# marl/l3embedding

Hardware: AMD Instinct MI355X
Metric: AVC training pairs/sec (1s audio + 224x224 frame) (higher is better)
Workload: dtype f32; 1 GPU; full cnn_L3_melspec2 AVC training step (audio+vision+fusion, fwd+bwd+Adam), batch 64 per GPU, global batch 64, fp32, inputs resident in HBM; global_batch=64, parallelism=dp1, fp32_conv=f4x4

## Files before the change

l3embedding_amd/csrc/conv_wgrad_bx6.hip:

```cpp
#include "kernels.h"
#include "device_common.h"
#include "wgw_common.h"

#include <stdlib.h>

#include <mutex>
#include <type_traits>

namespace l3 {

namespace {

template <int V>
using IC = std::integral_constant<int, V>;

__device__ __forceinline__ unsigned hi16_pair(unsigned a, unsigned b) { return __builtin_amdgcn_perm(b, a, 0x07060302u); }

struct Split3 {
    unsigned h, m, l;
};
__device__ __forceinline__ Split3 split_pair(float a, float b) {
    const unsigned ua = __builtin_bit_cast(unsigned, a), ub = __builtin_bit_cast(unsigned, b);
    Split3 s;
    s.h = hi16_pair(ua, ub);
    const float ra = a - __builtin_bit_cast(float, ua & 0xffff0000u), rb = b - __builtin_bit_cast(float, ub & 0xffff0000u);
    const unsigned va = __builtin_bit_cast(unsigned, ra), vb = __builtin_bit_cast(unsigned, rb);
    s.m = hi16_pair(va, vb);
    const float qa = ra - __builtin_bit_cast(float, va & 0xffff0000u), qb = rb - __builtin_bit_cast(float, vb & 0xffff0000u);
    s.l = hi16_pair(__builtin_bit_cast(unsigned, qa), __builtin_bit_cast(unsigned, qb));
    return s;
}

__device__ __forceinline__ f32x2 lds_pair(unsigned addr) {
    return *reinterpret_cast<const __attribute__((address_space(3))) f32x2*>((uintptr_t)addr);
}

template <int UC>
struct WgbGeom : WgwGeom<UC> {
    using G = WgwGeom<UC>;
    static constexpr int UNIT_BYTES = G::STAGE;
    static constexpr int STAGE2 = 2 * UNIT_BYTES;
    static constexpr unsigned BUF1 = 0x10000;
    static constexpr size_t LDS_BYTES = BUF1 + (size_t)STAGE2;
    static_assert(STAGE2 <= 0x10000, "stage buffer");
    static constexpr int PIECES2 = 2 * G::PIECES;
    static constexpr int PER_WAVE = (PIECES2 + 7) / 8;
    __host__ __device__ static constexpr int tr(int j) { return UC == 8 ? 0 : UC == 4 ? j >> 2 : j >> 1; }
    __host__ __device__ static constexpr int tc(int j) { return UC == 8 ? j : UC == 4 ? j & 3 : j & 1; }
};

template <int UC>
__global__ __launch_bounds__(512) void conv_wgrad_bx6_kernel(WgwArgs a) {
    using G = WgbGeom<UC>;
    constexpr int UR = G::UR, XPITCH = G::XPITCH, YPITCH = G::YPITCH, PER_WAVE = G::PER_WAVE;
    extern __shared__ __attribute__((aligned(16))) char smem[];

    const int t = threadIdx.x;
    const int wave = __builtin_amdgcn_readfirstlane(t >> 6), lane_id = t & 63;
    const int tiles = a.ctiles * a.ktiles;
    const int logical = xcd_remap(blockIdx.x, tiles * a.splits);
    const int sp = logical / tiles, tile = logical - sp * tiles;
    const int ct = tile / a.ktiles, kt = tile - ct * a.ktiles;
    const int c0 = ct * 64, k0 = kt * 64;
    const int u_begin = sp * a.per_split, u_end = min(a.units, u_begin + a.per_split);
    const int nunits = max(0, u_end - u_begin), nstage = (nunits + 1) >> 1;

    const int y_last = 2 * UR * (a.uy - 1), x_last = 2 * UC * (a.ux - 1);
    const size_t xshift = (size_t)(a.W + 1) * a.Cin * 4;
    const __amdgpu_buffer_rsrc_t xsrd = __builtin_amdgcn_make_buffer_rsrc(
        (void*)(reinterpret_cast<const char*>(a.x) - xshift), 0, (int)((size_t)a.N * a.H * a.W * a.Cin * 4 + xshift), 0x00020000);
    const __amdgpu_buffer_rsrc_t ysrd =
        __builtin_amdgcn_make_buffer_rsrc((void*)a.dy, 0, (int)((size_t)a.N * a.H * a.W * a.Cout * 4), 0x00020000);
    const int per_img = a.uy * a.ux;

    int q_u = u_begin;
    int q_n = u_begin / per_img, q_y = (u_begin - q_n * per_img) / a.ux, q_x = u_begin - q_n * per_img - q_y * a.ux;
    auto issue = [&](int s) __attribute__((always_inline)) {
        char* S = smem + (s & 1) * G::BUF1;
        int xbv[2], ybv[2];
        unsigned flg[2], dead[2];
#pragma unroll
        for (int h = 0; h < 2; ++h) {
            const int Y0 = 2 * UR * q_y, X0 = 2 * UC * q_x;
            xbv[h] = ((q_n * a.H + Y0) * a.W + X0) * a.Cin * 4;
            ybv[h] = ((q_n * a.H + Y0) * a.W + X0) * a.Cout * 4;
            flg[h] = (unsigned)(1 - min(q_y, 1)) | (unsigned)(1 - min(a.uy - 1 - q_y, 1)) << 1 | (unsigned)(1 - min(q_x, 1)) << 2 |
                     (unsigned)(1 - min(a.ux - 1 - q_x, 1)) << 3;
            dead[h] = q_u < u_end ? 0u : 0x80000000u;
            ++q_u;
            if (++q_x == a.ux) {
                q_x = 0;
                if (++q_y == a.uy) {
                    q_y = 0;
                    ++q_n;
                }
            }
        }
        int lane = lane_id;
        asm volatile("" : "+v"(lane));
#pragma unroll
        for (int q = 0; q < PER_WAVE; ++q) {
            const int pi = wave + 8 * q;
            if (pi < G::PIECES2) {
                const int h = pi >= G::PIECES ? 1 : 0;
                const int piece = pi - h * G::PIECES;
                const bool isx = piece < G::XPIECES;
                const int pix = (isx ? piece : piece - G::XPIECES) * 4 + (lane >> 4);
                const int py = isx ? pix / XPITCH : pix / YPITCH, px = isx ? pix - py * XPITCH : pix - py * YPITCH;
                const int ry = py - (isx ? 1 : 0), rx = px - (isx ? 1 : 0);
                const unsigned f = h ? flg[1] : flg[0];
                const unsigned out = ((f & 1u) & (unsigned)(ry < 0)) | ((f >> 1 & 1u) & (unsigned)(y_last + ry >= a.H)) |
                                     ((f >> 2 & 1u) & (unsigned)(rx < 0)) | ((f >> 3 & 1u) & (unsigned)(x_last + rx >= a.W)) |
                                     (unsigned)(isx && pix >= G::XPIX);
                const unsigned vo = (unsigned)((py * a.W + px) * (isx ? a.Cin : a.Cout) * 4 + (isx ? c0 : k0) * 4 + (lane & 15) * 16) |
                                    (out << 31) | (h ? dead[1] : dead[0]);
                auto* dst = (__attribute__((address_space(3))) void*)(S + h * G::UNIT_BYTES + piece * 1024);
                if (isx)
                    __builtin_amdgcn_raw_ptr_buffer_load_lds(xsrd, dst, 16, (int)vo, h ? xbv[1] : xbv[0], 0, 0);
                else
                    __builtin_amdgcn_raw_ptr_buffer_load_lds(ysrd, dst, 16, (int)vo, h ? ybv[1] : ybv[0], 0, 0);
            }
        }
    };

    const int l31 = lane_id & 31, grp = lane_id >> 5;
    const unsigned lds0 = (unsigned)(uintptr_t)smem;
    const unsigned lane_base = lds0 + (unsigned)(grp * G::UNIT_BYTES + l31 * 8);

    const int xi = wave >> 1;
    const int nuA = (wave & 1) ? 3 : 0, nuB = (wave & 1) ? 2 : 1;
    auto sgpr = [](float v) { return __builtin_bit_cast(float, __builtin_amdgcn_readfirstlane(__builtin_bit_cast(int, v))); };
    auto bt_a = [](int x) { return x == 0 ? 0 : x == 2 ? 2 : 1; };
    auto bt_b = [](int x) { return x == 0 ? 2 : x == 1 ? 2 : x == 2 ? 1 : 3; };
    const int ra = bt_a(xi), rb = bt_b(xi);
    const float sa = sgpr(xi == 1 ? 1.f : -1.f);
    const float sbA = sgpr(nuA == 1 ? 1.f : -1.f), sbB = sgpr(nuB == 1 ? 1.f : -1.f);
    const float r1 = sgpr(xi == 1 ? 1.f : -1.f), c1B = sgpr(nuB == 1 ? 1.f : -1.f);
    const int ry0 = xi == 3 ? 1 : 0, cy0A = nuA == 3 ? 1 : 0;
    auto xadr = [&](int r, int c) { return lane_base + (unsigned)((r * XPITCH + c) * 256); };
    auto yadr = [&](int r, int c) { return lane_base + (unsigned)(G::XBYTES + (r * YPITCH + c) * 256); };
    unsigned xA[4] = {xadr(ra, bt_a(nuA)), xadr(rb, bt_a(nuA)), xadr(ra, bt_b(nuA)), xadr(rb, bt_b(nuA))};
    unsigned xB[4] = {xadr(ra, bt_a(nuB)), xadr(rb, bt_a(nuB)), xadr(ra, bt_b(nuB)), xadr(rb, bt_b(nuB))};
    unsigned yA[2] = {yadr(ry0, cy0A), yadr(1, cy0A)};
    unsigned yB[4] = {yadr(ry0, 0), yadr(ry0, 1), yadr(1, 0), yadr(1, 1)};
    asm volatile("" : "+v"(xA[0]), "+v"(xA[1]), "+v"(xA[2]), "+v"(xA[3]), "+v"(xB[0]), "+v"(xB[1]), "+v"(xB[2]), "+v"(xB[3]));
    asm volatile("" : "+v"(yA[0]), "+v"(yA[1]), "+v"(yB[0]), "+v"(yB[1]), "+v"(yB[2]), "+v"(yB[3]));

    f32x16 acc[2][2][2];
#pragma unroll
    for (int pp = 0; pp < 2; ++pp)
#pragma unroll
        for (int i = 0; i < 2; ++i)
#pragma unroll
            for (int jn = 0; jn < 2; ++jn)
#pragma unroll
                for (int r = 0; r < 16; ++r) acc[pp][i][jn][r] = 0.f;

    auto run = [&](auto NRT, auto GRP) __attribute__((always_inline)) {
        constexpr int NR = decltype(NRT)::value;
        u32x4 Ah[2], Am[2], Al[2], Bh, Bm, Bl;
        auto lds_f = [](unsigned addr) { return *reinterpret_cast<const __attribute__((address_space(3))) float*>((uintptr_t)addr); };

        auto build_b = [&](auto PP, auto JN, unsigned buf) __attribute__((always_inline)) {
            constexpr int pp = decltype(PP)::value, jn = decltype(JN)::value;
            float z[2];
#pragma unroll
            for (int j = 0; j < 8; ++j) {
                if (!(j & 3)) __builtin_amdgcn_sched_barrier(0);
                const int tt = j & 1, tp = j >> 1;
                const unsigned yo = (unsigned)(((2 * G::tr(j)) * YPITCH + 2 * G::tc(j)) * 256 + 4 * jn);
                float zz;
                if constexpr (pp == 0) {
                    zz = lds_f(yA[0] + yo);
                    if constexpr (NR == 2) zz = fmaf(r1, lds_f(yA[1] + yo), zz);
                } else {
                    zz = fmaf(c1B, lds_f(yB[1] + yo), lds_f(yB[0] + yo));
                    if constexpr (NR == 2) zz = fmaf(r1, fmaf(c1B, lds_f(yB[3] + yo), lds_f(yB[2] + yo)), zz);
                }
                z[tt] = zz;
                if (tt == 1) {
                    const Split3 sz = split_pair(z[0], z[1]);
                    Bh[tp] = sz.h; Bm[tp] = sz.m; Bl[tp] = sz.l;
                }
            }
            __builtin_amdgcn_sched_barrier(0);
        };
        auto operands = [&](auto PP, unsigned buf) __attribute__((always_inline)) {
            constexpr int pp = decltype(PP)::value;
            const float sb = pp ? sbB : sbA;
            float v[2][2];
#pragma unroll
            for (int j = 0; j < 8; ++j) {
                if (!(j & 1)) __builtin_amdgcn_sched_barrier(0);
                const int tt = j & 1, tp = j >> 1;
                const unsigned xo = (unsigned)(((2 * G::tr(j)) * XPITCH + 2 * G::tc(j)) * 256);
                const f32x2 xa = lds_pair((pp ? xB[0] : xA[0]) + xo), xb = lds_pair((pp ? xB[1] : xA[1]) + xo);
                const f32x2 xc = lds_pair((pp ? xB[2] : xA[2]) + xo), xd = lds_pair((pp ? xB[3] : xA[3]) + xo);
#pragma unroll
                for (int e = 0; e < 2; ++e) v[tt][e] = fmaf(sb, fmaf(sa, xd[e], xc[e]), fmaf(sa, xb[e], xa[e]));
                if (tt == 1) {
#pragma unroll
                    for (int e = 0; e < 2; ++e) {
                        const Split3 sv = split_pair(v[0][e], v[1][e]);
                        Ah[e][tp] = sv.h; Am[e][tp] = sv.m; Al[e][tp] = sv.l;
                    }
                }
            }
            build_b(PP, IC<0>{}, buf);
        };
        auto multiply = [&](auto PP, unsigned buf) __attribute__((always_inline)) {
            constexpr int pp = decltype(PP)::value;
#pragma unroll
            for (int jn = 0; jn < 2; ++jn) {
                if (jn == 1) build_b(PP, IC<1>{}, buf);
                const bf16x8 bh = __builtin_bit_cast(bf16x8, Bh), bm = __builtin_bit_cast(bf16x8, Bm), bl = __builtin_bit_cast(bf16x8, Bl);
                const bf16x8 ah0 = __builtin_bit_cast(bf16x8, Ah[0]), am0 = __builtin_bit_cast(bf16x8, Am[0]), al0 = __builtin_bit_cast(bf16x8, Al[0]);
                const bf16x8 ah1 = __builtin_bit_cast(bf16x8, Ah[1]), am1 = __builtin_bit_cast(bf16x8, Am[1]), al1 = __builtin_bit_cast(bf16x8, Al[1]);
                f32x16 d0 = acc[pp][0][jn], d1 = acc[pp][1][jn];
                d0 = __builtin_amdgcn_mfma_f32_32x32x16_bf16(al0, bh, d0, 0, 0, 0);
                d1 = __builtin_amdgcn_mfma_f32_32x32x16_bf16(al1, bh, d1, 0, 0, 0);
                d0 = __builtin_amdgcn_mfma_f32_32x32x16_bf16(ah0, bl, d0, 0, 0, 0);
                d1 = __builtin_amdgcn_mfma_f32_32x32x16_bf16(ah1, bl, d1, 0, 0, 0);
                d0 = __builtin_amdgcn_mfma_f32_32x32x16_bf16(am0, bm, d0, 0, 0, 0);
                d1 = __builtin_amdgcn_mfma_f32_32x32x16_bf16(am1, bm, d1, 0, 0, 0);
                d0 = __builtin_amdgcn_mfma_f32_32x32x16_bf16(am0, bh, d0, 0, 0, 0);
                d1 = __builtin_amdgcn_mfma_f32_32x32x16_bf16(am1, bh, d1, 0, 0, 0);
                d0 = __builtin_amdgcn_mfma_f32_32x32x16_bf16(ah0, bm, d0, 0, 0, 0);
                d1 = __builtin_amdgcn_mfma_f32_32x32x16_bf16(ah1, bm, d1, 0, 0, 0);
                d0 = __builtin_amdgcn_mfma_f32_32x32x16_bf16(ah0, bh, d0, 0, 0, 0);
                d1 = __builtin_amdgcn_mfma_f32_32x32x16_bf16(ah1, bh, d1, 0, 0, 0);
                acc[pp][0][jn] = d0;
                acc[pp][1][jn] = d1;
                __builtin_amdgcn_sched_barrier(0);
            }
        };
        auto barrier = [] {
            __builtin_amdgcn_sched_barrier(0);
            __builtin_amdgcn_s_barrier();
            __builtin_amdgcn_sched_barrier(0);
        };
        auto wait_all = [] { asm volatile("s_waitcnt vmcnt(0)" ::: "memory"); };
        constexpr bool grp_o = decltype(GRP)::value != 0;
        if constexpr (grp_o) barrier();
        for (int c = 0; c < nstage; ++c) {
            const unsigned buf = 0;
            operands(IC<0>{}, buf);
            barrier();
            issue(c + 1);
            multiply(IC<0>{}, buf);
            barrier();
            operands(IC<1>{}, buf);
            if constexpr (grp_o) wait_all();
            barrier();
            multiply(IC<1>{}, buf);
            if constexpr (!grp_o) wait_all();
            barrier();
#pragma unroll
            for (int k = 0; k < 4; ++k) {
                xA[k] ^= G::BUF1;
                xB[k] ^= G::BUF1;
                yB[k] ^= G::BUF1;
            }
            yA[0] ^= G::BUF1;
            yA[1] ^= G::BUF1;
        }
        if constexpr (!grp_o) barrier();
    };
    {
        issue(0);
        asm volatile("s_waitcnt vmcnt(0)" ::: "memory");
        __syncthreads();
        const bool two_rows = xi == 1 || xi == 2;
        if (wave < 4) {
            if (two_rows) run(IC<2>{}, IC<0>{}); else run(IC<1>{}, IC<0>{});
        } else {
            if (two_rows) run(IC<2>{}, IC<1>{}); else run(IC<1>{}, IC<1>{});
        }
        asm volatile("s_waitcnt vmcnt(0)" ::: "memory");
    }

    int l31s = l31, grps = grp;
    asm volatile("" : "+v"(l31s), "+v"(grps));
#pragma unroll
    for (int pp = 0; pp < 2; ++pp) {
        const int nu = pp ? nuB : nuA;
        const float w00 = (xi == 3 ? -1.f : 1.f) * (nu == 3 ? -1.f : 1.f);
        float* out = a.part + ((size_t)(sp * 16 + xi * 4 + nu) * a.Cin + c0 + 8 * grps) * a.Cout + k0 + 2 * l31s;
#pragma unroll
        for (int i = 0; i < 2; ++i)
#pragma unroll
            for (int r = 0; r < 16; ++r) {
                const int c = 2 * ((r & 3) + 8 * (r >> 2)) + i;
                __builtin_nontemporal_store(f32x2{w00 * acc[pp][i][0][r], w00 * acc[pp][i][1][r]},
                                            reinterpret_cast<f32x2*>(out + (size_t)c * a.Cout));
            }
    }
}

template <int UC>
void launch_wgb(const WgwArgs& a, hipStream_t s) {
    using G = WgbGeom<UC>;
    static std::once_flag once[L3_MAX_DEVICES];
    int dev = 0;
    (void)hipGetDevice(&dev);
    std::call_once(once[dev & (L3_MAX_DEVICES - 1)], [] {
        (void)hipFuncSetAttribute((const void*)conv_wgrad_bx6_kernel<UC>, hipFuncAttributeMaxDynamicSharedMemorySize, (int)G::LDS_BYTES);
    });
    hipLaunchKernelGGL((conv_wgrad_bx6_kernel<UC>), dim3(a.ctiles * a.ktiles * a.splits), dim3(512), G::LDS_BYTES, s, a);
}

}

void conv_wgrad_bx6_launch(const WgwArgs& a, int uc, hipStream_t s) {
    if (uc == 8)
        launch_wgb<8>(a, s);
    else if (uc == 4)
        launch_wgb<4>(a, s);
    else
        launch_wgb<2>(a, s);
}

}
```

l3embedding_amd/csrc/conv_wgrad_wino.hip:

```cpp
#include "kernels.h"
#include "device_common.h"
#include "wgw_common.h"

#include <stdlib.h>

#include <mutex>

namespace l3 {

namespace {

__device__ __forceinline__ f32x2 lds_f32x2(unsigned lds_offset) {
    const f32x2 v = *reinterpret_cast<const __attribute__((address_space(3))) f32x2*>((uintptr_t)lds_offset);
    asm volatile("");
    return v;
}

__device__ __forceinline__ f32x2 pk_fma(f32x2 c, f32x2 x, f32x2 y) {
    asm("v_pk_fma_f32 %0, %1, %2, %0" : "+v"(y) : "s"(c), "v"(x));
    return y;
}
__device__ __forceinline__ f32x2 pk_fma_w(f32x2 c, f32x2 x, f32x2 y) {
    asm("v_pk_fma_f32 %0, %1, %2, %0\n\ts_nop 3" : "+v"(y) : "s"(c), "v"(x));
    return y;
}
template <int UC>
__global__ __launch_bounds__(1024) void conv_wgrad_wino_kernel(WgwArgs a) {
    using G = WgwGeom<UC>;
    constexpr int UR = G::UR, XPITCH = G::XPITCH, YPITCH = G::YPITCH;
    extern __shared__ __attribute__((aligned(16))) char smem[];

    const int t = threadIdx.x;
    const int wave = __builtin_amdgcn_readfirstlane(t >> 6), lane = t & 63;
    const int tiles = a.ctiles * a.ktiles;
    const int logical = xcd_remap(blockIdx.x, tiles * a.splits);
    const int sp = logical / tiles, tile = logical - sp * tiles;
    const int ct = tile / a.ktiles, kt = tile - ct * a.ktiles;
    const int c0 = ct * 64, k0 = kt * 64;
    const int u_begin = sp * a.per_split, u_end = min(a.units, u_begin + a.per_split);

    unsigned pc_voff[2], pc_out[2];
    bool pc_isx[2];
    const int y_last = 2 * UR * (a.uy - 1), x_last = 2 * UC * (a.ux - 1);
#pragma unroll
    for (int q = 0; q < 2; ++q) {
        const int piece = wave + 16 * q;
        const bool isx = piece < G::XPIECES;
        const int pix = (isx ? piece : piece - G::XPIECES) * 4 + (lane >> 4);
        const int pitch = isx ? XPITCH : YPITCH;
        const int py = pix / pitch, px = pix - py * pitch;
        const int C = isx ? a.Cin : a.Cout;
        const int ry = py - (isx ? 1 : 0), rx = px - (isx ? 1 : 0);
        pc_isx[q] = isx;
        pc_voff[q] = (unsigned)((py * a.W + px) * C * 4 + (isx ? c0 : k0) * 4 + (lane & 15) * 16);
        unsigned out = 0;
#pragma unroll
        for (int cls = 0; cls < 16; ++cls) {
            const int rc = cls >> 2, cc = cls & 3;
            const bool bad = ((rc & 1) && ry < 0) || ((rc & 2) && y_last + ry >= a.H) || ((cc & 1) && rx < 0) ||
                             ((cc & 2) && x_last + rx >= a.W) || (isx && pix >= G::XPIX);
            out |= bad ? 1u << cls : 0u;
        }
        pc_out[q] = out;
    }
    const bool second = wave + 16 < G::PIECES;
    const size_t xshift = (size_t)(a.W + 1) * a.Cin * 4;
    const __amdgpu_buffer_rsrc_t xsrd = __builtin_amdgcn_make_buffer_rsrc(
        (void*)(reinterpret_cast<const char*>(a.x) - xshift), 0, (int)((size_t)a.N * a.H * a.W * a.Cin * 4 + xshift), 0x00020000);
    const __amdgpu_buffer_rsrc_t ysrd =
        __builtin_amdgcn_make_buffer_rsrc((void*)a.dy, 0, (int)((size_t)a.N * a.H * a.W * a.Cout * 4), 0x00020000);

    const int per_img = a.uy * a.ux;
    int un = u_begin / per_img;
    int uyi = (u_begin - un * per_img) / a.ux;
    int uxi = u_begin - un * per_img - uyi * a.ux;

    auto issue = [&](int buf) {
        const int Y0 = 2 * UR * uyi, X0 = 2 * UC * uxi;
        const int xbase = ((un * a.H + Y0) * a.W + X0) * a.Cin * 4;
        const int ybase = ((un * a.H + Y0) * a.W + X0) * a.Cout * 4;
        const int rcls = (1 - min(uyi, 1)) + 2 * (1 - min(a.uy - 1 - uyi, 1)), ccls = (1 - min(uxi, 1)) + 2 * (1 - min(a.ux - 1 - uxi, 1));
        const int cls = rcls * 4 + ccls;
        char* S = smem + buf * G::STAGE;
#pragma unroll
        for (int q = 0; q < 2; ++q) {
            if (q == 1 && !second) break;
            const unsigned vo = (__builtin_amdgcn_ubfe(pc_out[q], (unsigned)cls, 1u) << 31) | pc_voff[q];
            if (pc_isx[q])
                __builtin_amdgcn_raw_ptr_buffer_load_lds(xsrd, (__attribute__((address_space(3))) void*)(S + (wave + 16 * q) * 1024),
                                                         16, (int)vo, xbase, 0, 0);
            else
                __builtin_amdgcn_raw_ptr_buffer_load_lds(ysrd, (__attribute__((address_space(3))) void*)(S + (wave + 16 * q) * 1024),
                                                         16, (int)vo, ybase, 0, 0);
        }
        if (++uxi == a.ux) {
            uxi = 0;
            if (++uyi == a.uy) {
                uyi = 0;
                ++un;
            }
        }
    };

    const int xi = wave >> 2, nu = (wave + (wave >> 2)) & 3;
    const int ra = xi == 0 ? 0 : xi == 2 ? 2 : 1, rb = xi == 0 ? 2 : xi == 1 ? 2 : xi == 2 ? 1 : 3;
    const int ca = nu == 0 ? 0 : nu == 2 ? 2 : 1, cb = nu == 0 ? 2 : nu == 1 ? 2 : nu == 2 ? 1 : 3;
    auto sgpr = [](float v) { return __builtin_bit_cast(float, __builtin_amdgcn_readfirstlane(__builtin_bit_cast(int, v))); };
    const float sa = sgpr(xi == 1 ? 1.f : -1.f), sb = sgpr(nu == 1 ? 1.f : -1.f);
    const int nr = (xi == 0 || xi == 3) ? 1 : 2, nc = (nu == 0 || nu == 3) ? 1 : 2;
    const int ry0 = xi == 3 ? 1 : 0, cy0 = nu == 3 ? 1 : 0;
    const float sr0 = xi == 3 ? -1.f : 1.f, sr1 = xi == 2 ? -1.f : 1.f;
    const float sc0 = nu == 3 ? -1.f : 1.f, sc1 = nu == 2 ? -1.f : 1.f;
    const float w00 = sgpr(sr0 * sc0), w01 = sgpr(sr0 * sc1), w10 = sgpr(sr1 * sc0), w11 = sgpr(sr1 * sc1);
    const f32x2 sa2 = {sa, sa}, sb2 = {sb, sb}, w01_2 = {w01 * w00, w01 * w00}, w10_2 = {w10 * w00, w10 * w00},
                w11_2 = {w11 * w00, w11 * w00};

    const int l31 = lane & 31, half = lane >> 5;
    const int ltr = G::lane_tr(half), ltc = G::lane_tc(half);
    auto xaddr = [&](int r, int c) { return ((r + 2 * ltr) * XPITCH + c + 2 * ltc) * 256 + l31 * 8; };
    auto yaddr = [&](int r, int c) { return G::XBYTES + ((r + 2 * ltr) * YPITCH + c + 2 * ltc) * 256 + l31 * 8; };
    const int x_aa = xaddr(ra, ca), x_ba = xaddr(rb, ca), x_ab = xaddr(ra, cb), x_bb = xaddr(rb, cb);
    const int y_00 = yaddr(ry0, cy0), y_01 = yaddr(ry0, 1), y_10 = yaddr(1, cy0), y_11 = yaddr(1, 1);
    const unsigned lds0 = (unsigned)(uintptr_t)smem;
    unsigned p_aa = lds0 + x_aa, p_ba = lds0 + x_ba, p_ab = lds0 + x_ab, p_bb = lds0 + x_bb;
    unsigned q_00 = lds0 + y_00, q_01 = lds0 + y_01, q_10 = lds0 + y_10, q_11 = lds0 + y_11;
    asm volatile("" : "+v"(p_aa), "+v"(p_ba), "+v"(p_ab), "+v"(p_bb), "+v"(q_00), "+v"(q_01), "+v"(q_10), "+v"(q_11));

    f32x16 acc[2][2];
#pragma unroll
    for (int i = 0; i < 2; ++i)
#pragma unroll
        for (int jn = 0; jn < 2; ++jn)
#pragma unroll
            for (int r = 0; r < 16; ++r) acc[i][jn][r] = 0.f;

    struct Raw {
        f32x2 x[4], y[4];
    };
    auto run = [&](auto NRT, auto NCT) {
    constexpr int NR = decltype(NRT)::value, NC = decltype(NCT)::value;
    auto load_raw = [&](int sb, auto JT, Raw& r, const Raw& prev) {
        constexpr int j = decltype(JT)::value;
        constexpr bool share = NC == 1 && j > 0 && G::imm_tr(j) == G::imm_tr(j > 0 ? j - 1 : 0) &&
                               G::imm_tc(j) == G::imm_tc(j > 0 ? j - 1 : 0) + 1;
        const int ix = ((2 * G::imm_tr(j)) * XPITCH + 2 * G::imm_tc(j)) * 256;
        const int iy = ((2 * G::imm_tr(j)) * YPITCH + 2 * G::imm_tc(j)) * 256;
        f32x2 xa, xb;
        if constexpr (share) {
            xa = prev.x[2];
            xb = prev.x[3];
        } else {
            xa = lds_f32x2(p_aa + sb + ix);
            xb = lds_f32x2(p_ba + sb + ix);
        }
        const f32x2 xc = lds_f32x2(p_ab + sb + ix), xd = lds_f32x2(p_bb + sb + ix);
        f32x2 ya = lds_f32x2(q_00 + sb + iy), yb = ya, yc = ya, yd = ya;
        if (NC == 2) yb = lds_f32x2(q_01 + sb + iy);
        if (NR == 2) yc = lds_f32x2(q_10 + sb + iy);
        if (NR == 2 && NC == 2) yd = lds_f32x2(q_11 + sb + iy);
        r.x[0] = xa; r.x[1] = xb; r.x[2] = xc; r.x[3] = xd;
        r.y[0] = ya; r.y[1] = yb; r.y[2] = yc; r.y[3] = yd;
    };
    auto mfma_step = [&](const Raw& r) {
        const f32x2 v = pk_fma_w(sb2, pk_fma(sa2, r.x[3], r.x[2]), pk_fma(sa2, r.x[1], r.x[0]));
        f32x2 z;
        if constexpr (NR == 1 && NC == 1) {
            z = r.y[0];
        } else if constexpr (NR == 1) {
            z = pk_fma_w(w01_2, r.y[1], r.y[0]);
        } else if constexpr (NC == 1) {
            z = pk_fma_w(w10_2, r.y[2], r.y[0]);
        } else {
            z = pk_fma_w(w11_2, r.y[3], pk_fma(w10_2, r.y[2], pk_fma(w01_2, r.y[1], r.y[0])));
        }
#pragma unroll
        for (int i = 0; i < 2; ++i)
#pragma unroll
            for (int jn = 0; jn < 2; ++jn) acc[i][jn] = __builtin_amdgcn_mfma_f32_32x32x2f32(v[i], z[jn], acc[i][jn], 0, 0, 0);
    };
    auto compute = [&](auto BUF) {
        constexpr int S = decltype(BUF)::value * G::STAGE;
        Raw r0, r1;
        load_raw(S, std::integral_constant<int, 0>{}, r0, r0);
        __builtin_amdgcn_sched_barrier(0);
        load_raw(S, std::integral_constant<int, 1>{}, r1, r0);
        mfma_step(r0);
        __builtin_amdgcn_sched_barrier(0);
        load_raw(S, std::integral_constant<int, 2>{}, r0, r1);
        mfma_step(r1);
        __builtin_amdgcn_sched_barrier(0);
        load_raw(S, std::integral_constant<int, 3>{}, r1, r0);
        mfma_step(r0);
        __builtin_amdgcn_sched_barrier(0);
        mfma_step(r1);
    };
    auto stage_barrier = [&]() {
        __builtin_amdgcn_sched_barrier(0);
        __syncthreads();
        __builtin_amdgcn_sched_barrier(0);
    };

    const int nunits = u_end - u_begin;
    if (nunits > 0) {
        issue(0);
        __syncthreads();
        for (int u = 0; u < nunits; u += 2) {
            if (u + 1 < nunits) issue(1);
            compute(std::integral_constant<int, 0>{});
            stage_barrier();
            if (u + 1 < nunits) {
                if (u + 2 < nunits) issue(0);
                compute(std::integral_constant<int, 1>{});
                stage_barrier();
            }
        }
    }
    };
    if (nr == 1 && nc == 1)
        run(std::integral_constant<int, 1>{}, std::integral_constant<int, 1>{});
    else if (nr == 1)
        run(std::integral_constant<int, 1>{}, std::integral_constant<int, 2>{});
    else if (nc == 1)
        run(std::integral_constant<int, 2>{}, std::integral_constant<int, 1>{});
    else
        run(std::integral_constant<int, 2>{}, std::integral_constant<int, 2>{});

    float* out = a.part + ((size_t)(sp * 16 + xi * 4 + nu) * a.Cin + c0) * a.Cout + k0;
#pragma unroll
    for (int i = 0; i < 2; ++i)
#pragma unroll
        for (int r = 0; r < 16; ++r) {
            const int c = 2 * ((r & 3) + 8 * (r >> 2) + 4 * half) + i;
            __builtin_nontemporal_store(f32x2{w00 * acc[i][0][r], w00 * acc[i][1][r]}, reinterpret_cast<f32x2*>(out + (size_t)c * a.Cout + 2 * l31));
        }
}

__global__ __launch_bounds__(256) void wgw_finish_kernel(const float* __restrict__ part, float* __restrict__ dw, int cc,
                                                         int splits) {
    const int idx = blockIdx.x * 256 + threadIdx.x;
    if (idx >= cc) return;
    float u[16];
#pragma unroll
    for (int p = 0; p < 16; ++p) u[p] = 0.f;
    for (int s = 0; s < splits; ++s)
#pragma unroll
        for (int p = 0; p < 16; ++p) u[p] += __builtin_nontemporal_load(part + ((size_t)s * 16 + p) * cc + idx);
    float rrow[3][4];
#pragma unroll
    for (int nu = 0; nu < 4; ++nu) {
        const float h1 = 0.5f * u[4 + nu], h2 = 0.5f * u[8 + nu];
        rrow[0][nu] = u[nu] + (h1 + h2);
        rrow[1][nu] = h1 - h2;
        rrow[2][nu] = (h1 + h2) + u[12 + nu];
    }
#pragma unroll
    for (int kh = 0; kh < 3; ++kh) {
        const float h1 = 0.5f * rrow[kh][1], h2 = 0.5f * rrow[kh][2];
        dw[(size_t)(kh * 3 + 0) * cc + idx] = rrow[kh][0] + (h1 + h2);
        dw[(size_t)(kh * 3 + 1) * cc + idx] = h1 - h2;
        dw[(size_t)(kh * 3 + 2) * cc + idx] = (h1 + h2) + rrow[kh][3];
    }
}

struct WgwPlan {
    int uc, uy, ux, units, per_split, splits;
};

WgwPlan wgw_plan(const ConvGeom& g, int n, int force_uc = 0) {
    const int TY = (g.H + 1) / 2, TX = (g.W + 1) / 2;
    WgwPlan p;
    size_t best = ~(size_t)0;
    p.uc = 8;
    for (int uc : {8, 4, 2}) {
        const int ur = 8 / uc;
        const size_t padded = (size_t)((TY + ur - 1) / ur * ur) * ((TX + uc - 1) / uc * uc);
        if (padded < best) {
            best = padded;
            p.uc = uc;
        }
    }
    const char* fenv = l3_knob("L3_WGW_UC");
    const int force = force_uc ? force_uc : fenv ? atoi(fenv) : 0;
    if (force == 8 || force == 4 || force == 2) p.uc = force;
    const int ur = 8 / p.uc;
    p.uy = (TY + ur - 1) / ur;
    p.ux = (TX + p.uc - 1) / p.uc;
    p.units = n * p.uy * p.ux;
    const int tiles = (g.Cin / 64) * (g.Cout / 64);
    static const int target = l3_knob("L3_WGW_BLOCKS") ? atoi(l3_knob("L3_WGW_BLOCKS")) : 256;
    int splits = (target + tiles - 1) / tiles;
    const int max_splits = (p.units + 31) / 32;
    if (splits > max_splits) splits = max_splits;
    if (splits < 1) splits = 1;
    p.per_split = (p.units + splits - 1) / splits;
    p.splits = (p.units + p.per_split - 1) / p.per_split;
    return p;
}

template <int UC>
void launch_wgw(const WgwArgs& a, hipStream_t s) {
    using G = WgwGeom<UC>;
    static std::once_flag once[L3_MAX_DEVICES];
    int dev = 0;
    (void)hipGetDevice(&dev);
    std::call_once(once[dev & (L3_MAX_DEVICES - 1)], [] {
        (void)hipFuncSetAttribute((const void*)conv_wgrad_wino_kernel<UC>, hipFuncAttributeMaxDynamicSharedMemorySize,
                                  (int)G::LDS_BYTES);
    });
    hipLaunchKernelGGL((conv_wgrad_wino_kernel<UC>), dim3(a.ctiles * a.ktiles * a.splits), dim3(1024), G::LDS_BYTES, s, a);
}

}

bool conv_wgrad_wino_ok(const ConvGeom& g) {
    const char* env = l3_knob("L3_WG_WINO");
    return (env ? atoi(env) : 1) && g.KH == 3 && g.KW == 3 && g.padT == 1 && g.padL == 1 && g.Ho == g.H && g.Wo == g.W &&
           g.Cin % 64 == 0 && g.Cout % 64 == 0;
}

int conv_wgrad_wino_splits(const ConvGeom& g, int n) { return wgw_plan(g, n).splits; }

int conv_wgrad_wino_max_splits(const ConvGeom& g, int n) {
    int m = wgw_plan(g, n).splits;
    for (int uc : {8, 4, 2}) {
        const int sp = wgw_plan(g, n, uc).splits;
        if (sp > m) m = sp;
    }
    return m;
}

double conv_wgrad_wino_executed_flops(const ConvGeom& g) {
    const WgwPlan p = wgw_plan(g, g.N);
    return 2.0 * 16.0 * (double)p.units * 8.0 * (double)g.Cin * (double)g.Cout;
}

void conv_wgrad_wino_launch(const float* x, const float* dy, float* part, const ConvGeom& g, int n, hipStream_t s) {
    const WgwPlan p = wgw_plan(g, n);
    WgwArgs a;
    a.x = x; a.dy = dy; a.part = part;
    a.N = n; a.H = g.H; a.W = g.W; a.Cin = g.Cin; a.Cout = g.Cout;
    a.uy = p.uy; a.ux = p.ux; a.units = p.units; a.per_split = p.per_split; a.splits = p.splits;
    a.ctiles = g.Cin / 64; a.ktiles = g.Cout / 64;
#ifdef L3_EXPERIMENTS
    const char* bx = l3_knob("L3_WG_BX6");
    if (bx != nullptr && atoi(bx) == 1) return conv_wgrad_bx6_launch(a, p.uc, s);
#endif
    if (p.uc == 8)
        launch_wgw<8>(a, s);
    else if (p.uc == 4)
        launch_wgw<4>(a, s);
    else
        launch_wgw<2>(a, s);
}

void conv_wgrad_wino_finish(const float* part, float* dw, const ConvGeom& g, int splits, hipStream_t s) {
    const int cc = g.Cin * g.Cout;
    hipLaunchKernelGGL(wgw_finish_kernel, dim3((cc + 255) / 256), dim3(256), 0, s, part, dw, cc, splits);
}

}
```

l3embedding_amd/csrc/wgw_common.h:

```cpp
#pragma once
#include "kernels.h"
#include "device_common.h"

namespace l3 {

struct WgwArgs {
    const float* x;
    const float* dy;
    float* part;
    int N, H, W, Cin, Cout;
    int uy, ux;
    int units;
    int per_split, splits;
    int ctiles, ktiles;
};

template <int UC>
struct WgwGeom {
    static constexpr int UR = 8 / UC;
    static constexpr int XROWS = 2 * UR + 2, XPITCH = 2 * UC + 2, XPIX = XROWS * XPITCH;
    static constexpr int YPITCH = 2 * UC, YPIX = 32;
    static constexpr int XPIECES = (XPIX + 3) / 4;
    static constexpr int YPIECES = YPIX / 4;
    static constexpr int PIECES = XPIECES + YPIECES;
    static constexpr int XBYTES = XPIECES * 1024;
    static constexpr int STAGE = PIECES * 1024;
    static constexpr size_t LDS_BYTES = 2 * (size_t)STAGE;
    static_assert(PIECES <= 32, "two pieces per wave at most");
    __host__ __device__ static constexpr int lane_tr(int half) { return UC == 8 ? 0 : UC == 4 ? half : 2 * half; }
    __host__ __device__ static constexpr int lane_tc(int half) { return UC == 8 ? 4 * half : 0; }
    __host__ __device__ static constexpr int imm_tr(int j) { return UC == 2 ? j >> 1 : 0; }
    __host__ __device__ static constexpr int imm_tc(int j) { return UC == 2 ? j & 1 : j; }
};

void conv_wgrad_bx6_launch(const WgwArgs& a, int uc, hipStream_t s);

}
```

Baseline: 2053 pairs/s.

## Add 2x5 and 2x7 Winograd wgrad unit shapes to reduce spatial padding

Generalizes the Winograd weight-gradient kernel from fixed 8-tile units (1x8, 2x4, 4x2) to templated UR x UC shapes, adding 2x5, 2x7 and 2x8 variants. The planner picks the shape that minimizes padded tile count, so feature maps whose tile grid is not a multiple of 8 waste less work. It also generalizes the per-wave piece count (up to three) and the k-step loop via a static_for. Larger units use more LDS per stage and more load pieces per wave, which may reduce occupancy or change the pipeline balance.

```diff
diff --git a/l3embedding_amd/csrc/conv_wgrad_bx6.hip b/l3embedding_amd/csrc/conv_wgrad_bx6.hip
--- a/l3embedding_amd/csrc/conv_wgrad_bx6.hip
+++ b/l3embedding_amd/csrc/conv_wgrad_bx6.hip
@@ -36,8 +36,8 @@
 }
 
 template <int UC>
-struct WgbGeom : WgwGeom<UC> {
-    using G = WgwGeom<UC>;
+struct WgbGeom : WgwGeom<8 / UC, UC> {
+    using G = WgwGeom<8 / UC, UC>;
     static constexpr int UNIT_BYTES = G::STAGE;
     static constexpr int STAGE2 = 2 * UNIT_BYTES;
     static constexpr unsigned BUF1 = 0x10000;
diff --git a/l3embedding_amd/csrc/conv_wgrad_wino.hip b/l3embedding_amd/csrc/conv_wgrad_wino.hip
--- a/l3embedding_amd/csrc/conv_wgrad_wino.hip
+++ b/l3embedding_amd/csrc/conv_wgrad_wino.hip
@@ -24,10 +24,18 @@
     asm("v_pk_fma_f32 %0, %1, %2, %0\n\ts_nop 3" : "+v"(y) : "s"(c), "v"(x));
     return y;
 }
-template <int UC>
+template <int B, int E, class F>
+__device__ __forceinline__ void static_for(F&& f) {
+    if constexpr (B < E) {
+        f(std::integral_constant<int, B>{});
+        static_for<B + 1, E>(f);
+    }
+}
+
+template <int UR, int UC>
 __global__ __launch_bounds__(1024) void conv_wgrad_wino_kernel(WgwArgs a) {
-    using G = WgwGeom<UC>;
-    constexpr int UR = G::UR, XPITCH = G::XPITCH, YPITCH = G::YPITCH;
+    using G = WgwGeom<UR, UC>;
+    constexpr int XPITCH = G::XPITCH, YPITCH = G::YPITCH, PW = G::PER_WAVE;
     extern __shared__ __attribute__((aligned(16))) char smem[];
 
     const int t = threadIdx.x;
@@ -39,11 +47,11 @@
     const int c0 = ct * 64, k0 = kt * 64;
     const int u_begin = sp * a.per_split, u_end = min(a.units, u_begin + a.per_split);
 
-    unsigned pc_voff[2], pc_out[2];
-    bool pc_isx[2];
+    unsigned pc_voff[PW], pc_out[PW];
+    bool pc_isx[PW];
     const int y_last = 2 * UR * (a.uy - 1), x_last = 2 * UC * (a.ux - 1);
 #pragma unroll
-    for (int q = 0; q < 2; ++q) {
+    for (int q = 0; q < PW; ++q) {
         const int piece = wave + 16 * q;
         const bool isx = piece < G::XPIECES;
         const int pix = (isx ? piece : piece - G::XPIECES) * 4 + (lane >> 4);
@@ -63,7 +71,7 @@
         }
         pc_out[q] = out;
     }
-    const bool second = wave + 16 < G::PIECES;
+    const bool last = wave + 16 * (PW - 1) < G::PIECES;
     const size_t xshift = (size_t)(a.W + 1) * a.Cin * 4;
     const __amdgpu_buffer_rsrc_t xsrd = __builtin_amdgcn_make_buffer_rsrc(
         (void*)(reinterpret_cast<const char*>(a.x) - xshift), 0, (int)((size_t)a.N * a.H * a.W * a.Cin * 4 + xshift), 0x00020000);
@@ -83,8 +91,8 @@
         const int cls = rcls * 4 + ccls;
         char* S = smem + buf * G::STAGE;
 #pragma unroll
-        for (int q = 0; q < 2; ++q) {
-            if (q == 1 && !second) break;
+        for (int q = 0; q < PW; ++q) {
+            if (q == PW - 1 && !last) break;
             const unsigned vo = (__builtin_amdgcn_ubfe(pc_out[q], (unsigned)cls, 1u) << 31) | pc_voff[q];
             if (pc_isx[q])
                 __builtin_amdgcn_raw_ptr_buffer_load_lds(xsrd, (__attribute__((address_space(3))) void*)(S + (wave + 16 * q) * 1024),
@@ -183,16 +191,17 @@
         Raw r0, r1;
         load_raw(S, std::integral_constant<int, 0>{}, r0, r0);
         __builtin_amdgcn_sched_barrier(0);
-        load_raw(S, std::integral_constant<int, 1>{}, r1, r0);
-        mfma_step(r0);
-        __builtin_amdgcn_sched_barrier(0);
-        load_raw(S, std::integral_constant<int, 2>{}, r0, r1);
-        mfma_step(r1);
-        __builtin_amdgcn_sched_barrier(0);
-        load_raw(S, std::integral_constant<int, 3>{}, r1, r0);
-        mfma_step(r0);
-        __builtin_amdgcn_sched_barrier(0);
-        mfma_step(r1);
+        static_for<1, G::KSTEPS>([&](auto JT) {
+            if constexpr (decltype(JT)::value & 1) {
+                load_raw(S, JT, r1, r0);
+                mfma_step(r0);
+            } else {
+                load_raw(S, JT, r0, r1);
+                mfma_step(r1);
+            }
+            __builtin_amdgcn_sched_barrier(0);
+        });
+        mfma_step(G::KSTEPS & 1 ? r0 : r1);
     };
     auto stage_barrier = [&]() {
         __builtin_amdgcn_sched_barrier(0);
@@ -262,28 +271,50 @@
     }
 }
 
+struct WgwShape {
+    int ur, uc;
+};
+constexpr WgwShape kShapes[] = {{1, 8}, {2, 4}, {4, 2}, {2, 5}, {2, 7}, {2, 8}};
+constexpr int kLegacyShapes = 3, kPlannedShapes = 5, kShapeCount = 6;
+
 struct WgwPlan {
-    int uc, uy, ux, units, per_split, splits;
+    int shape, ur, uc, uy, ux, units, per_split, splits;
 };
 
-WgwPlan wgw_plan(const ConvGeom& g, int n, int force_uc = 0) {
+int wgw_forced_shape() {
+    const char* fenv = l3_knob("L3_WGW_UC");
+    const int v = fenv ? atoi(fenv) : 0;
+    return v == 8 ? 0 : v == 4 ? 1 : v == 2 ? 2 : v == 5 ? 3 : v == 7 ? 4 : v == 28 ? 5 : -1;
+}
+
+bool wgw_bx6() {
+#ifdef L3_EXPERIMENTS
+    const char* bx = l3_knob("L3_WG_BX6");
+    return bx != nullptr && atoi(bx) == 1;
+#else
+    return false;
+#endif
+}
+
+WgwPlan wgw_plan(const ConvGeom& g, int n, int force_shape = -1) {
     const int TY = (g.H + 1) / 2, TX = (g.W + 1) / 2;
+    const bool legacy_only = wgw_bx6();
     WgwPlan p;
     size_t best = ~(size_t)0;
-    p.uc = 8;
-    for (int uc : {8, 4, 2}) {
-        const int ur = 8 / uc;
+    p.shape = 0;
+    for (int i = 0; i < (legacy_only ? kLegacyShapes : kPlannedShapes); ++i) {
+        const int ur = kShapes[i].ur, uc = kShapes[i].uc;
         const size_t padded = (size_t)((TY + ur - 1) / ur * ur) * ((TX + uc - 1) / uc * uc);
         if (padded < best) {
             best = padded;
-            p.uc = uc;
-        }
-    }
-    const char* fenv = l3_knob("L3_WGW_UC");
-    const int force = force_uc ? force_uc : fenv ? atoi(fenv) : 0;
-    if (force == 8 || force == 4 || force == 2) p.uc = force;
-    const int ur = 8 / p.uc;
-    p.uy = (TY + ur - 1) / ur;
+            p.shape = i;
+        }
+    }
+    const int force = force_shape >= 0 ? force_shape : wgw_forced_shape();
+    if (force >= 0 && force < (legacy_only ? kLegacyShapes : kShapeCount)) p.shape = force;
+    p.ur = kShapes[p.shape].ur;
+    p.uc = kShapes[p.shape].uc;
+    p.uy = (TY + p.ur - 1) / p.ur;
     p.ux = (TX + p.uc - 1) / p.uc;
     p.units = n * p.uy * p.ux;
     const int tiles = (g.Cin / 64) * (g.Cout / 64);
@@ -297,17 +328,17 @@
     return p;
 }
 
-template <int UC>
+template <int UR, int UC>
 void launch_wgw(const WgwArgs& a, hipStream_t s) {
-    using G = WgwGeom<UC>;
+    using G = WgwGeom<UR, UC>;
     static std::once_flag once[L3_MAX_DEVICES];
     int dev = 0;
     (void)hipGetDevice(&dev);
     std::call_once(once[dev & (L3_MAX_DEVICES - 1)], [] {
-        (void)hipFuncSetAttribute((const void*)conv_wgrad_wino_kernel<UC>, hipFuncAttributeMaxDynamicSharedMemorySize,
+        (void)hipFuncSetAttribute((const void*)conv_wgrad_wino_kernel<UR, UC>, hipFuncAttributeMaxDynamicSharedMemorySize,
                                   (int)G::LDS_BYTES);
     });
-    hipLaunchKernelGGL((conv_wgrad_wino_kernel<UC>), dim3(a.ctiles * a.ktiles * a.splits), dim3(1024), G::LDS_BYTES, s, a);
+    hipLaunchKernelGGL((conv_wgrad_wino_kernel<UR, UC>), dim3(a.ctiles * a.ktiles * a.splits), dim3(1024), G::LDS_BYTES, s, a);
 }
 
 }
@@ -322,8 +353,8 @@
 
 int conv_wgrad_wino_max_splits(const ConvGeom& g, int n) {
     int m = wgw_plan(g, n).splits;
-    for (int uc : {8, 4, 2}) {
-        const int sp = wgw_plan(g, n, uc).splits;
+    for (int i = 0; i < kShapeCount; ++i) {
+        const int sp = wgw_plan(g, n, i).splits;
         if (sp > m) m = sp;
     }
     return m;
@@ -331,7 +362,7 @@
 
 double conv_wgrad_wino_executed_flops(const ConvGeom& g) {
     const WgwPlan p = wgw_plan(g, g.N);
-    return 2.0 * 16.0 * (double)p.units * 8.0 * (double)g.Cin * (double)g.Cout;
+    return 2.0 * 16.0 * (double)p.units * (double)(p.ur * p.uc) * (double)g.Cin * (double)g.Cout;
 }
 
 void conv_wgrad_wino_launch(const float* x, const float* dy, float* part, const ConvGeom& g, int n, hipStream_t s) {
@@ -342,15 +373,16 @@
     a.uy = p.uy; a.ux = p.ux; a.units = p.units; a.per_split = p.per_split; a.splits = p.splits;
     a.ctiles = g.Cin / 64; a.ktiles = g.Cout / 64;
 #ifdef L3_EXPERIMENTS
-    const char* bx = l3_knob("L3_WG_BX6");
-    if (bx != nullptr && atoi(bx) == 1) return conv_wgrad_bx6_launch(a, p.uc, s);
+    if (wgw_bx6()) return conv_wgrad_bx6_launch(a, p.uc, s);
 #endif
-    if (p.uc == 8)
-        launch_wgw<8>(a, s);
-    else if (p.uc == 4)
-        launch_wgw<4>(a, s);
-    else
-        launch_wgw<2>(a, s);
+    switch (p.shape) {
+        case 0: return launch_wgw<1, 8>(a, s);
+        case 1: return launch_wgw<2, 4>(a, s);
+        case 2: return launch_wgw<4, 2>(a, s);
+        case 3: return launch_wgw<2, 5>(a, s);
+        case 4: return launch_wgw<2, 7>(a, s);
+        default: return launch_wgw<2, 8>(a, s);
+    }
 }
 
 void conv_wgrad_wino_finish(const float* part, float* dw, const ConvGeom& g, int splits, hipStream_t s) {
diff --git a/l3embedding_amd/csrc/wgw_common.h b/l3embedding_amd/csrc/wgw_common.h
--- a/l3embedding_amd/csrc/wgw_common.h
+++ b/l3embedding_amd/csrc/wgw_common.h
@@ -15,22 +15,27 @@
     int ctiles, ktiles;
 };
 
-template <int UC>
+template <int UR_, int UC_>
 struct WgwGeom {
-    static constexpr int UR = 8 / UC;
+    static constexpr int UR = UR_, UC = UC_;
+    static_assert(UR * UC % 2 == 0 && (UR == 2 || UR * UC == 8), "1x8, 4x2 or two tile rows");
+    static constexpr int KSTEPS = UR * UC / 2;
     static constexpr int XROWS = 2 * UR + 2, XPITCH = 2 * UC + 2, XPIX = XROWS * XPITCH;
-    static constexpr int YPITCH = 2 * UC, YPIX = 32;
+    static constexpr int YPITCH = 2 * UC, YPIX = 4 * UR * UC;
     static constexpr int XPIECES = (XPIX + 3) / 4;
     static constexpr int YPIECES = YPIX / 4;
     static constexpr int PIECES = XPIECES + YPIECES;
+    static constexpr int PER_WAVE = (PIECES + 15) / 16;
     static constexpr int XBYTES = XPIECES * 1024;
     static constexpr int STAGE = PIECES * 1024;
     static constexpr size_t LDS_BYTES = 2 * (size_t)STAGE;
-    static_assert(PIECES <= 32, "two pieces per wave at most");
-    __host__ __device__ static constexpr int lane_tr(int half) { return UC == 8 ? 0 : UC == 4 ? half : 2 * half; }
-    __host__ __device__ static constexpr int lane_tc(int half) { return UC == 8 ? 4 * half : 0; }
-    __host__ __device__ static constexpr int imm_tr(int j) { return UC == 2 ? j >> 1 : 0; }
-    __host__ __device__ static constexpr int imm_tc(int j) { return UC == 2 ? j & 1 : j; }
+    static_assert(PER_WAVE <= 3, "three pieces per wave at most");
+    __host__ __device__ static constexpr int lane_tr(int half) { return UR == 1 ? 0 : UR == 2 ? half : 2 * half; }
+    __host__ __device__ static constexpr int lane_tc(int half) { return UR == 1 ? 4 * half : 0; }
+    __host__ __device__ static constexpr int imm_tr(int j) { return UR == 4 ? j >> 1 : 0; }
+    __host__ __device__ static constexpr int imm_tc(int j) { return UR == 4 ? j & 1 : j; }
+    static constexpr int MAX_IMM = STAGE + (2 * imm_tr(KSTEPS - 1) * XPITCH + 2 * imm_tc(KSTEPS - 1)) * 256;
+    static_assert(MAX_IMM < 65536, "DS immediate offset");
 };
 
 void conv_wgrad_bx6_launch(const WgwArgs& a, int uc, hipStream_t s);
```

After: 2068 pairs/s (median of 6 runs). About the same (+0.7%).
